# matter-labs/era-boojum

Measured on AMD Instinct MI355X. Metric: prover_constraints_per_sec, higher is better.
Workload: dtype u64

## Files before the change

### era_boojum_amd/csrc/stage2.hip

```cpp
#include "gl.h"
#include "kernels.h"

using gl::u64;
using gl::u32;

namespace bj {

static constexpr int RAT_PTS = 4;
template <bool SMALLK>
__global__ void __launch_bounds__(256)
copy_perm_rational_kernel(const u64 *vars, size_t var_stride, const u64 *sigmas, size_t sig_stride, const u64 *non_res,
                          unsigned V, unsigned chunk, unsigned log_n, const u64 *tw, gl::e2 beta, gl::e2 gamma, u64 *out) {
    const size_t n = (size_t)1 << log_n;
    const size_t base = (size_t)blockIdx.x * (256 * RAT_PTS) + threadIdx.x;
    const unsigned j = blockIdx.y;
    gl::e2 num[RAT_PTS], den[RAT_PTS];
    u64 xb0[RAT_PTS], xb1[RAT_PTS];
#pragma unroll
    for (int k = 0; k < RAT_PTS; k++) {
        const size_t r = base + (size_t)k * 256;
        const u64 x = r < n ? gl::omega_pow_nat(tw, log_n, (u32)r) : 0;
        xb0[k] = gl::mul_weak(x, beta.c0);
        xb1[k] = gl::mul_weak(x, beta.c1);
        num[k] = {1, 0};
        den[k] = {1, 0};
    }
    for (unsigned i = j * chunk; i < (j + 1) * chunk && i < V; i++) {
        const u64 kr = SMALLK ? gl::canon(non_res[i]) : non_res[i];
#pragma unroll
        for (int k = 0; k < RAT_PTS; k++) {
            const size_t r = base + (size_t)k * 256;
            if (r >= n) continue;
            const u64 w = vars[(size_t)i * var_stride + r];
            const u64 wg = gl::add_weak(w, gamma.c0);
            const gl::e2 a = SMALLK ? gl::e2{gl::add_weak(gl::mul_u32_weak(xb0[k], (u32)kr), wg), gl::add_weak(gl::mul_u32_weak(xb1[k], (u32)kr), gamma.c1)}
                                    : gl::e2{gl::add_weak(gl::mul_weak(kr, xb0[k]), wg), gl::add_weak(gl::mul_weak(kr, xb1[k]), gamma.c1)};
            const u64 s = sigmas[(size_t)i * sig_stride + r];
            const gl::e2 b{gl::add_weak(gl::mul_weak(s, beta.c0), wg), gl::add_weak(gl::mul_weak(s, beta.c1), gamma.c1)};
            num[k] = gl::e2_mul_weak(num[k], a);
            den[k] = gl::e2_mul_weak(den[k], b);
        }
    }
#pragma unroll
    for (int k = 0; k < RAT_PTS; k++) {
        num[k] = {gl::canon(num[k].c0), gl::canon(num[k].c1)};
        den[k] = {gl::canon(den[k].c0), gl::canon(den[k].c1)};
    }
    gl::e2 pre[RAT_PTS], run{1, 0};
#pragma unroll
    for (int k = 0; k < RAT_PTS; k++) {
        pre[k] = run;
        run = gl::e2_mul(run, den[k]);
    }
    gl::e2 inv_run = gl::e2_inv_chain(run);
#pragma unroll
    for (int k = RAT_PTS - 1; k >= 0; k--) {
        const gl::e2 inv_k = gl::e2_mul(inv_run, pre[k]);
        inv_run = gl::e2_mul(inv_run, den[k]);
        const size_t r = base + (size_t)k * 256;
        if (r < n) {
            gl::e2 p = gl::e2_mul(num[k], inv_k);
            out[((size_t)2 * j) * n + r] = p.c0;
            out[((size_t)2 * j + 1) * n + r] = p.c1;
        }
    }
}

__global__ void __launch_bounds__(256) chunk_prefix_kernel(u64 *P, unsigned n_chunks, size_t n) {
    const size_t r = (size_t)blockIdx.x * blockDim.x + threadIdx.x;
    if (r >= n) return;
    gl::e2 acc{P[r], P[n + r]};
    for (unsigned j = 1; j < n_chunks; j++) {
        gl::e2 p{P[((size_t)2 * j) * n + r], P[((size_t)2 * j + 1) * n + r]};
        acc = gl::e2_mul(acc, p);
        P[((size_t)2 * j) * n + r] = acc.c0;
        P[((size_t)2 * j + 1) * n + r] = acc.c1;
    }
}

static constexpr int SCAN_TPB = 256, SCAN_PER_THREAD = 4, SCAN_BLOCK = SCAN_TPB * SCAN_PER_THREAD;

__device__ __forceinline__ gl::e2 block_exclusive_scan(gl::e2 v, gl::e2 *lds, gl::e2 &total) {
    const unsigned t = threadIdx.x;
    lds[t] = v;
    __syncthreads();
    for (unsigned off = 1; off < SCAN_TPB; off <<= 1) {
        gl::e2 cur = lds[t];
        gl::e2 other = t >= off ? lds[t - off] : gl::e2{1, 0};
        __syncthreads();
        lds[t] = t >= off ? gl::e2_mul(other, cur) : cur;
        __syncthreads();
    }
    total = lds[SCAN_TPB - 1];
    gl::e2 excl = t ? lds[t - 1] : gl::e2{1, 0};
    __syncthreads();
    return excl;
}

__global__ void __launch_bounds__(SCAN_TPB)
scan_local_kernel(const u64 *a0, const u64 *a1, u64 *z0, u64 *z1, u64 *block_tot, size_t n) {
    __shared__ gl::e2 lds[SCAN_TPB];
    const size_t base = (size_t)blockIdx.x * SCAN_BLOCK + (size_t)threadIdx.x * SCAN_PER_THREAD;
    gl::e2 v[SCAN_PER_THREAD], pre[SCAN_PER_THREAD];
    gl::e2 run{1, 0};
#pragma unroll
    for (int k = 0; k < SCAN_PER_THREAD; k++) {
        size_t r = base + k;
        v[k] = r < n ? gl::e2{a0[r], a1[r]} : gl::e2{1, 0};
        pre[k] = run;
        run = gl::e2_mul(run, v[k]);
    }
    gl::e2 total;
    gl::e2 excl = block_exclusive_scan(run, lds, total);
#pragma unroll
    for (int k = 0; k < SCAN_PER_THREAD; k++) {
        size_t r = base + k;
        if (r < n) {
            gl::e2 o = gl::e2_mul(excl, pre[k]);
            z0[r] = o.c0;
            z1[r] = o.c1;
        }
    }
    if (threadIdx.x == 0) {
        block_tot[2 * (size_t)blockIdx.x] = total.c0;
        block_tot[2 * (size_t)blockIdx.x + 1] = total.c1;
    }
}
__global__ void __launch_bounds__(SCAN_TPB) scan_blocks_kernel(u64 *block_tot, size_t n_blocks) {
    __shared__ gl::e2 lds[SCAN_TPB];
    gl::e2 carry{1, 0};
    for (size_t start = 0; start < n_blocks; start += SCAN_TPB) {
        size_t i = start + threadIdx.x;
        gl::e2 v = i < n_blocks ? gl::e2{block_tot[2 * i], block_tot[2 * i + 1]} : gl::e2{1, 0};
        gl::e2 total;
        gl::e2 excl = block_exclusive_scan(v, lds, total);
        if (i < n_blocks) {
            gl::e2 o = gl::e2_mul(carry, excl);
            block_tot[2 * i] = o.c0;
            block_tot[2 * i + 1] = o.c1;
        }
        carry = gl::e2_mul(carry, total);
        __syncthreads();
    }
}
__global__ void __launch_bounds__(256)
scan_apply_partials_kernel(u64 *z0, u64 *z1, const u64 *block_pre, const u64 *Q, unsigned n_chunks, size_t n,
                           u64 *partials ) {
    const size_t r = (size_t)blockIdx.x * blockDim.x + threadIdx.x;
    if (r >= n) return;
    size_t b = r / SCAN_BLOCK;
    gl::e2 z = gl::e2_mul(gl::e2{block_pre[2 * b], block_pre[2 * b + 1]}, gl::e2{z0[r], z1[r]});
    z0[r] = z.c0;
    z1[r] = z.c1;
    for (unsigned k = 0; k + 1 < n_chunks; k++) {
        gl::e2 qk{Q[((size_t)2 * k) * n + r], Q[((size_t)2 * k + 1) * n + r]};
        gl::e2 p = gl::e2_mul(z, qk);
        partials[((size_t)2 * k) * n + r] = p.c0;
        partials[((size_t)2 * k + 1) * n + r] = p.c1;
    }
}

void launch_copy_perm_stage2(const u64 *d_vars, size_t var_stride, const u64 *d_sigmas, size_t sig_stride,
                             const u64 *d_non_res, unsigned V, unsigned chunk, unsigned log_n, const u64 *d_tw_fwd,
                             const u64 *beta, const u64 *gamma, u64 *d_tmp, u64 *d_z, u64 *d_partials, hipStream_t s,
                             bool small_non_residues) {
    const size_t n = (size_t)1 << log_n;
    const unsigned n_chunks = (V + chunk - 1) / chunk;
    gl::e2 b{gl::canon(beta[0]), gl::canon(beta[1])}, g{gl::canon(gamma[0]), gl::canon(gamma[1])};
    u64 *P = d_tmp;
    u64 *block_tot = d_tmp + (size_t)2 * n_chunks * n;
    const unsigned rb = (unsigned)((n + 255) / 256);
    if (small_non_residues && !env().copy_perm_wide_k)
        hipLaunchKernelGGL(copy_perm_rational_kernel<true>, dim3((unsigned)((n + 256 * RAT_PTS - 1) / (256 * RAT_PTS)), n_chunks), dim3(256), 0, s, d_vars, var_stride,
                           d_sigmas, sig_stride, d_non_res, V, chunk, log_n, d_tw_fwd, b, g, P);
    else
        hipLaunchKernelGGL(copy_perm_rational_kernel<false>, dim3((unsigned)((n + 256 * RAT_PTS - 1) / (256 * RAT_PTS)), n_chunks), dim3(256), 0, s, d_vars, var_stride,
                           d_sigmas, sig_stride, d_non_res, V, chunk, log_n, d_tw_fwd, b, g, P);
    hipLaunchKernelGGL(chunk_prefix_kernel, dim3(rb), dim3(256), 0, s, P, n_chunks, n);
    const u64 *a0 = P + ((size_t)2 * (n_chunks - 1)) * n, *a1 = a0 + n;
    const size_t n_blocks = (n + SCAN_BLOCK - 1) / SCAN_BLOCK;
    hipLaunchKernelGGL(scan_local_kernel, dim3((unsigned)n_blocks), dim3(SCAN_TPB), 0, s, a0, a1, d_z, d_z + n, block_tot, n);
    hipLaunchKernelGGL(scan_blocks_kernel, dim3(1), dim3(SCAN_TPB), 0, s, block_tot, n_blocks);
    hipLaunchKernelGGL(scan_apply_partials_kernel, dim3(rb), dim3(256), 0, s, d_z, d_z + n, block_tot, P, n_chunks, n,
                       d_partials);
}

struct LookupArgs {
    gl::e2 beta;
    gl::e2 gpow[9];
};
__global__ void __launch_bounds__(256)
lookup_polys_kernel(const u64 *lvars, size_t var_stride, const u64 *table_id, const u64 *tables, size_t tab_stride,
                    const u64 *mult, unsigned reps, unsigned w, size_t n, LookupArgs a, u64 *outA, u64 *outB) {
    const size_t r = (size_t)blockIdx.x * blockDim.x + threadIdx.x;
    if (r >= n) return;
    const unsigned cps = table_id ? w : w + 1;
    const u64 tid = table_id ? gl::canon(table_id[r]) : 0;
    constexpr unsigned LK_GROUP = 9;
    for (unsigned g0 = 0; g0 <= reps; g0 += LK_GROUP) {
        const unsigned cnt = (reps + 1 - g0) < LK_GROUP ? (reps + 1 - g0) : LK_GROUP;
        gl::e2 den[LK_GROUP], pre[LK_GROUP], run{1, 0};
#pragma unroll
        for (unsigned k = 0; k < LK_GROUP; k++) {
            if (k >= cnt) break;
            const unsigned i = g0 + k;
            gl::e2 acc = a.beta;
            if (i < reps) {
                for (unsigned j = 0; j < cps; j++) {
                    u64 v = gl::canon(lvars[(size_t)(i * cps + j) * var_stride + r]);
                    acc = gl::e2_add(acc, gl::e2_mul_base(a.gpow[j], v));
                }
                if (table_id) acc = gl::e2_add(acc, gl::e2_mul_base(a.gpow[w], tid));
            } else {
                for (unsigned j = 0; j <= w; j++) {
                    u64 v = gl::canon(tables[(size_t)j * tab_stride + r]);
                    acc = gl::e2_add(acc, gl::e2_mul_base(a.gpow[j], v));
                }
            }
            den[k] = acc;
            pre[k] = run;
            run = gl::e2_mul(run, acc);
        }
        gl::e2 inv_run = gl::e2_inv_chain(run);
#pragma unroll
        for (int k = (int)LK_GROUP - 1; k >= 0; k--) {
            if ((unsigned)k >= cnt) continue;
            const unsigned i = g0 + (unsigned)k;
            const gl::e2 inv = gl::e2_mul(inv_run, pre[k]);
            inv_run = gl::e2_mul(inv_run, den[k]);
            if (i < reps) {
                outA[((size_t)2 * i) * n + r] = inv.c0;
                outA[((size_t)2 * i + 1) * n + r] = inv.c1;
            } else {
                gl::e2 bb = gl::e2_mul_base(inv, gl::canon(mult[r]));
                outB[r] = bb.c0;
                outB[n + r] = bb.c1;
            }
        }
    }
}

void launch_lookup_polys(const u64 *d_lvars, size_t var_stride, const u64 *d_table_id, const u64 *d_tables,
                         size_t tab_stride, const u64 *d_mult, unsigned reps, unsigned w, unsigned log_n,
                         const u64 *beta, const u64 *gamma, u64 *d_A, u64 *d_B, hipStream_t s) {
    const size_t n = (size_t)1 << log_n;
    LookupArgs a;
    a.beta = {gl::canon(beta[0]), gl::canon(beta[1])};
    gl::e2 g{gl::canon(gamma[0]), gl::canon(gamma[1])};
    a.gpow[0] = {1, 0};
    for (unsigned j = 1; j <= w && j < 9; j++) a.gpow[j] = gl::e2_mul(a.gpow[j - 1], g);
    hipLaunchKernelGGL(lookup_polys_kernel, dim3((unsigned)((n + 255) / 256)), dim3(256), 0, s, d_lvars, var_stride,
                       d_table_id, d_tables, tab_stride, d_mult, reps, w, n, a, d_A, d_B);
}

}
```

Baseline: 16.76 million.

## Fuse copy-permutation rational and chunk prefix into one per-row kernel

Replaces the per-chunk rational kernel plus the separate chunk_prefix pass with one kernel in which each thread handles a whole row. The thread first runs a backward pass over the denominators and stores suffix products in LDS and register slots. It then takes a single inversion and runs a forward pass over the numerators, writing the chunk prefix ratios directly. This removes one inversion per chunk, one kernel launch, and the global read-modify-write of the prefix pass. In exchange it loses the 2D chunk parallelism and the 4-point batched inversion, reads each variable column twice, and relies on a large register and LDS footprint with launch bounds set to 3 waves.

```diff
diff --git a/era_boojum_amd/csrc/stage2.hip b/era_boojum_amd/csrc/stage2.hip
--- a/era_boojum_amd/csrc/stage2.hip
+++ b/era_boojum_amd/csrc/stage2.hip
@@ -1,81 +1,78 @@
 #include "gl.h"
 #include "kernels.h"
+#include "stage2_row.h"
 
 using gl::u64;
 using gl::u32;
 
 namespace bj {
 
-static constexpr int RAT_PTS = 4;
+static constexpr unsigned S2_LDS_SLOTS = 13, S2_REG_SLOTS = 17, S2_SLOTS = S2_LDS_SLOTS + S2_REG_SLOTS;
+#define BJ_S2_REG_CASES(X) X(0) X(1) X(2) X(3) X(4) X(5) X(6) X(7) X(8) X(9) X(10) X(11) X(12) X(13) X(14) X(15) X(16)
+struct RowCols {
+    const u64 *vars, *sigmas, *non_res;
+    size_t var_stride, sig_stride;
+    bool smallk;
+    __device__ __forceinline__ u64 var(unsigned i) const { return vars[(size_t)i * var_stride]; }
+    __device__ __forceinline__ u64 sigma(unsigned i) const { return sigmas[(size_t)i * sig_stride]; }
+    __device__ __forceinline__ u64 k(unsigned i) const { return smallk ? gl::canon(non_res[i]) : non_res[i]; }
+};
+struct RowSlots {
+    u64 *lds;
+    u64 *P;
+    size_t n;
+    gl::e2 reg[S2_REG_SLOTS];
+    __device__ __forceinline__ void put(unsigned j, gl::e2 v) {
+        if (j < S2_LDS_SLOTS) {
+            lds[(2 * j) * 256] = v.c0;
+            lds[(2 * j + 1) * 256] = v.c1;
+        } else if (j < S2_SLOTS) {
+            switch (j - S2_LDS_SLOTS) {
+#define X(k) case k: reg[k] = v; break;
+                BJ_S2_REG_CASES(X)
+#undef X
+            }
+        } else {
+            P[((size_t)2 * j) * n] = v.c0;
+            P[((size_t)2 * j + 1) * n] = v.c1;
+        }
+    }
+    __device__ __forceinline__ gl::e2 get(unsigned j) const {
+        if (j < S2_LDS_SLOTS) return {lds[(2 * j) * 256], lds[(2 * j + 1) * 256]};
+        if (j < S2_SLOTS) {
+            switch (j - S2_LDS_SLOTS) {
+#define X(k) case k: return reg[k];
+                BJ_S2_REG_CASES(X)
+#undef X
+            }
+        }
+        return {P[((size_t)2 * j) * n], P[((size_t)2 * j + 1) * n]};
+    }
+};
+#undef BJ_S2_REG_CASES
+struct RowOut {
+    u64 *P;
+    size_t n;
+    __device__ __forceinline__ void operator()(unsigned j, gl::e2 p) const {
+        P[((size_t)2 * j) * n] = p.c0;
+        P[((size_t)2 * j + 1) * n] = p.c1;
+    }
+};
 template <bool SMALLK>
-__global__ void __launch_bounds__(256)
-copy_perm_rational_kernel(const u64 *vars, size_t var_stride, const u64 *sigmas, size_t sig_stride, const u64 *non_res,
-                          unsigned V, unsigned chunk, unsigned log_n, const u64 *tw, gl::e2 beta, gl::e2 gamma, u64 *out) {
+__global__ void __launch_bounds__(256, 3)
+copy_perm_prefix_kernel(const u64 *vars, size_t var_stride, const u64 *sigmas, size_t sig_stride, const u64 *non_res,
+                        unsigned V, unsigned chunk, unsigned log_n, const u64 *tw, gl::e2 beta, gl::e2 gamma, u64 *out) {
+    __shared__ u64 lds[S2_LDS_SLOTS * 2 * 256];
     const size_t n = (size_t)1 << log_n;
-    const size_t base = (size_t)blockIdx.x * (256 * RAT_PTS) + threadIdx.x;
-    const unsigned j = blockIdx.y;
-    gl::e2 num[RAT_PTS], den[RAT_PTS];
-    u64 xb0[RAT_PTS], xb1[RAT_PTS];
-#pragma unroll
-    for (int k = 0; k < RAT_PTS; k++) {
-        const size_t r = base + (size_t)k * 256;
-        const u64 x = r < n ? gl::omega_pow_nat(tw, log_n, (u32)r) : 0;
-        xb0[k] = gl::mul_weak(x, beta.c0);
-        xb1[k] = gl::mul_weak(x, beta.c1);
-        num[k] = {1, 0};
-        den[k] = {1, 0};
-    }
-    for (unsigned i = j * chunk; i < (j + 1) * chunk && i < V; i++) {
-        const u64 kr = SMALLK ? gl::canon(non_res[i]) : non_res[i];
-#pragma unroll
-        for (int k = 0; k < RAT_PTS; k++) {
-            const size_t r = base + (size_t)k * 256;
-            if (r >= n) continue;
-            const u64 w = vars[(size_t)i * var_stride + r];
-            const u64 wg = gl::add_weak(w, gamma.c0);
-            const gl::e2 a = SMALLK ? gl::e2{gl::add_weak(gl::mul_u32_weak(xb0[k], (u32)kr), wg), gl::add_weak(gl::mul_u32_weak(xb1[k], (u32)kr), gamma.c1)}
-                                    : gl::e2{gl::add_weak(gl::mul_weak(kr, xb0[k]), wg), gl::add_weak(gl::mul_weak(kr, xb1[k]), gamma.c1)};
-            const u64 s = sigmas[(size_t)i * sig_stride + r];
-            const gl::e2 b{gl::add_weak(gl::mul_weak(s, beta.c0), wg), gl::add_weak(gl::mul_weak(s, beta.c1), gamma.c1)};
-            num[k] = gl::e2_mul_weak(num[k], a);
-            den[k] = gl::e2_mul_weak(den[k], b);
-        }
-    }
-#pragma unroll
-    for (int k = 0; k < RAT_PTS; k++) {
-        num[k] = {gl::canon(num[k].c0), gl::canon(num[k].c1)};
-        den[k] = {gl::canon(den[k].c0), gl::canon(den[k].c1)};
-    }
-    gl::e2 pre[RAT_PTS], run{1, 0};
-#pragma unroll
-    for (int k = 0; k < RAT_PTS; k++) {
-        pre[k] = run;
-        run = gl::e2_mul(run, den[k]);
-    }
-    gl::e2 inv_run = gl::e2_inv_chain(run);
-#pragma unroll
-    for (int k = RAT_PTS - 1; k >= 0; k--) {
-        const gl::e2 inv_k = gl::e2_mul(inv_run, pre[k]);
-        inv_run = gl::e2_mul(inv_run, den[k]);
-        const size_t r = base + (size_t)k * 256;
-        if (r < n) {
-            gl::e2 p = gl::e2_mul(num[k], inv_k);
-            out[((size_t)2 * j) * n + r] = p.c0;
-            out[((size_t)2 * j + 1) * n + r] = p.c1;
-        }
-    }
-}
-
-__global__ void __launch_bounds__(256) chunk_prefix_kernel(u64 *P, unsigned n_chunks, size_t n) {
-    const size_t r = (size_t)blockIdx.x * blockDim.x + threadIdx.x;
+    const size_t r = (size_t)blockIdx.x * 256 + threadIdx.x;
     if (r >= n) return;
-    gl::e2 acc{P[r], P[n + r]};
-    for (unsigned j = 1; j < n_chunks; j++) {
-        gl::e2 p{P[((size_t)2 * j) * n + r], P[((size_t)2 * j + 1) * n + r]};
-        acc = gl::e2_mul(acc, p);
-        P[((size_t)2 * j) * n + r] = acc.c0;
-        P[((size_t)2 * j + 1) * n + r] = acc.c1;
-    }
+    const RowCols cols{vars + r, sigmas + r, non_res, var_stride, sig_stride, SMALLK};
+    RowSlots slots;
+    slots.lds = lds + threadIdx.x;
+    slots.P = out + r;
+    slots.n = n;
+    RowOut put{out + r, n};
+    copy_perm_row_prefixes<SMALLK>(cols, V, chunk, gl::omega_pow_nat(tw, log_n, (u32)r), beta, gamma, slots, put);
 }
 
 static constexpr int SCAN_TPB = 256, SCAN_PER_THREAD = 4, SCAN_BLOCK = SCAN_TPB * SCAN_PER_THREAD;
@@ -171,12 +168,11 @@
     u64 *block_tot = d_tmp + (size_t)2 * n_chunks * n;
     const unsigned rb = (unsigned)((n + 255) / 256);
     if (small_non_residues && !env().copy_perm_wide_k)
-        hipLaunchKernelGGL(copy_perm_rational_kernel<true>, dim3((unsigned)((n + 256 * RAT_PTS - 1) / (256 * RAT_PTS)), n_chunks), dim3(256), 0, s, d_vars, var_stride,
-                           d_sigmas, sig_stride, d_non_res, V, chunk, log_n, d_tw_fwd, b, g, P);
+        hipLaunchKernelGGL(copy_perm_prefix_kernel<true>, dim3(rb), dim3(256), 0, s, d_vars, var_stride, d_sigmas, sig_stride, d_non_res, V, chunk, log_n,
+                           d_tw_fwd, b, g, P);
     else
-        hipLaunchKernelGGL(copy_perm_rational_kernel<false>, dim3((unsigned)((n + 256 * RAT_PTS - 1) / (256 * RAT_PTS)), n_chunks), dim3(256), 0, s, d_vars, var_stride,
-                           d_sigmas, sig_stride, d_non_res, V, chunk, log_n, d_tw_fwd, b, g, P);
-    hipLaunchKernelGGL(chunk_prefix_kernel, dim3(rb), dim3(256), 0, s, P, n_chunks, n);
+        hipLaunchKernelGGL(copy_perm_prefix_kernel<false>, dim3(rb), dim3(256), 0, s, d_vars, var_stride, d_sigmas, sig_stride, d_non_res, V, chunk, log_n,
+                           d_tw_fwd, b, g, P);
     const u64 *a0 = P + ((size_t)2 * (n_chunks - 1)) * n, *a1 = a0 + n;
     const size_t n_blocks = (n + SCAN_BLOCK - 1) / SCAN_BLOCK;
     hipLaunchKernelGGL(scan_local_kernel, dim3((unsigned)n_blocks), dim3(SCAN_TPB), 0, s, a0, a1, d_z, d_z + n, block_tot, n);
diff --git a/era_boojum_amd/csrc/stage2_row.h b/era_boojum_amd/csrc/stage2_row.h
--- /dev/null
+++ b/era_boojum_amd/csrc/stage2_row.h
@@ -0,0 +1,54 @@
+#pragma once
+#include "gl.h"
+
+namespace bj {
+
+template <bool SMALLK, class Cols, class Slots, class Out>
+__host__ __device__ __forceinline__ void copy_perm_row_prefixes(const Cols &cols, unsigned V, unsigned chunk, gl::u64 x, gl::e2 beta, gl::e2 gamma,
+                                                                Slots &slots, Out &out) {
+    using gl::u64;
+    using gl::u32;
+    const unsigned n_chunks = (V + chunk - 1) / chunk;
+    gl::e2 run{1, 0};
+    {
+        unsigned j = n_chunks - 1, left = V - j * chunk;
+        u64 w = cols.var(V - 1), s = cols.sigma(V - 1);
+        for (unsigned i = V; i-- > 0;) {
+            u64 wn = w, sn = s;
+            if (i > 0) {
+                wn = cols.var(i - 1);
+                sn = cols.sigma(i - 1);
+            }
+            const u64 wg = gl::add_weak(w, gamma.c0);
+            const gl::e2 b{gl::add_weak(gl::mul_weak(s, beta.c0), wg), gl::add_weak(gl::mul_weak(s, beta.c1), gamma.c1)};
+            run = gl::e2_mul_weak(run, b);
+            if (--left == 0 && j > 0) {
+                slots.put(--j, run);
+                left = chunk;
+            }
+            w = wn;
+            s = sn;
+        }
+    }
+    gl::e2 num = gl::e2_inv_chain({gl::canon(run.c0), gl::canon(run.c1)});
+    const u64 xb0 = gl::mul_weak(x, beta.c0), xb1 = gl::mul_weak(x, beta.c1);
+    unsigned j = 0, left = chunk;
+    u64 w = cols.var(0);
+    for (unsigned i = 0; i < V; i++) {
+        const u64 wn = i + 1 < V ? cols.var(i + 1) : w;
+        const u64 kr = cols.k(i);
+        const u64 wg = gl::add_weak(w, gamma.c0);
+        const gl::e2 a = SMALLK ? gl::e2{gl::add_weak(gl::mul_u32_weak(xb0, (u32)kr), wg), gl::add_weak(gl::mul_u32_weak(xb1, (u32)kr), gamma.c1)}
+                                : gl::e2{gl::add_weak(gl::mul_weak(kr, xb0), wg), gl::add_weak(gl::mul_weak(kr, xb1), gamma.c1)};
+        num = gl::e2_mul_weak(num, a);
+        if (--left == 0 || i + 1 == V) {
+            const gl::e2 p = j + 1 < n_chunks ? gl::e2_mul_weak(num, slots.get(j)) : num;
+            out(j, gl::e2{gl::canon(p.c0), gl::canon(p.c1)});
+            j++;
+            left = chunk;
+        }
+        w = wn;
+    }
+}
+
+}
```

Measured after the change: 16.83 million (median of 6 runs). Within noise of the previous version (+0.4%).
